# forestagostinelli/DeepCubeA

Measured on AMD Instinct MI355X. Metric: A* nodes expanded/sec on cube3, batch 20k, higher is better.
Workload: dtype u8 states / f64 cost keys / f32 heuristic

## Files before the change

deepcubea_amd/csrc/dca_engine.hip:

```cpp
#include <string.h>

#include <new>
#include <vector>

#include "dca_common.h"
#include "dca_tile.h"

namespace dca {

constexpr int NBIN = 4096;
constexpr int kBinsPerThread = NBIN / 1024;
constexpr int kLgNbin = 12;
constexpr int kSub = 2048;
constexpr int kScanBlocks = 256;
constexpr int kCollectBlocks = 512;
constexpr int kRankBlocks = 256;
constexpr uint32_t kTinyBin = 512;
constexpr int kSortCap = 8192;
constexpr int RT = 512;
constexpr int kRegEnt = 16;
constexpr uint32_t kLdsEnt = RT * kRegEnt;
constexpr int kStash = 2560;
constexpr int kSegs = NBIN + 1 + kSub;
constexpr uint32_t kGiantBin = 8192;
constexpr int kMaxLevels = 9;
constexpr unsigned long long kBarrierTimeout = 200000000ull;
constexpr unsigned long long kBarrierTimeoutFirst = 25000000ull;
constexpr uint32_t GBAR_BROKEN = 0x80000000u;
constexpr uint32_t NIL = 0xFFFFFFFFu;
constexpr uint32_t ID_MASK = 0x7FFFFFFFu, ID_SOLVED = 0x80000000u;
constexpr uint64_t EMPTY = ~0ull;
constexpr uint64_t DEAD = ~0ull;
constexpr uint32_t GINF = 0xFFFFFFFFu;
constexpr int kMaxMoves = 4096;

struct Slot {
    uint64_t entry;
    uint32_t g;
    uint32_t head;
};

struct alignas(128) Cnt {
    uint32_t v;
    uint32_t pad[31];
};
struct alignas(128) GRange {
    uint64_t kmin, kmax;
    uint32_t imin, imax;
    uint32_t pad[26];
};
struct alignas(128) Rng {
    uint64_t kmin, kmax;
    uint64_t pad[14];
};
struct IterState {
    uint32_t pool_n;
    uint32_t npop, m, base;
    uint32_t best_id;
    int32_t has_best;
    float best_cost;
};
struct Ctl {
    int32_t done, failed, stop_after, pad0;
    int64_t iters, gen, expanded;
    IterState S[2];
    uint32_t cur_f;
    uint32_t hbin;
    uint32_t front_above;
    uint32_t cur_b;
    uint64_t T;
    uint32_t refill, compact, r_bstar, spill_bin, r_move;
    uint64_t r_kmin;
    uint32_t r_shift;
    uint32_t want, bstar, shift, n_big, n_ord;
    uint32_t giant;
    uint32_t tseg;
    uint32_t pre_b, cn_star;
    uint64_t sel_kmin;
    uint32_t goal_id;
    uint32_t dbg_nord, dbg_maxbin, dbg_giant, dbg_giant_seen, dbg_maxsub;
    Cnt open_n[4];
    Cnt closed_n, back_dead, front_dead, ret_n, ticket_a;
    Cnt gbar;
    GRange grange;
    Rng rng[4];
    alignas(128) unsigned long long goal_best;
    alignas(128) uint32_t first_solved;
};

__device__ __forceinline__ uint64_t key_of_cost(double c) {
    uint64_t b = (uint64_t)__double_as_longlong(c);
    return (b & 0x8000000000000000ull) ? ~b : (b | 0x8000000000000000ull);
}
__device__ __forceinline__ double cost_of_key(uint64_t k) {
    uint64_t b = (k & 0x8000000000000000ull) ? (k & 0x7FFFFFFFFFFFFFFFull) : ~k;
    return __longlong_as_double((long long)b);
}
__device__ __forceinline__ uint32_t select_shift(uint64_t kmin, uint64_t kmax) {
    uint64_t range = kmax - kmin;
    int bits = range ? 64 - __clzll((long long)range) : 0;
    return bits > kLgNbin ? (uint32_t)(bits - kLgNbin) : 0u;
}
__device__ __forceinline__ uint32_t bin_of(uint64_t k, uint64_t kmin, uint32_t shift) {
    if (k <= kmin) return 0u;
    const uint64_t f = (k - kmin) >> shift;
    return f < (uint64_t)NBIN ? (uint32_t)f : (uint32_t)(NBIN - 1);
}
__device__ __forceinline__ bool pair_less(uint64_t ka, uint32_t ia, uint64_t kb, uint32_t ib) {
    return ka < kb || (ka == kb && (ia & ID_MASK) < (ib & ID_MASK));
}

enum {
    P_REFILL_HIST = 0, P_REFILL_SCAN, P_REFILL_MOVE, P_SEL_HIST, P_SEL_SCAN, P_SEL_COLLECT, P_RANK, P_EXPAND,
    P_PROBE,
    P_DECIDE, P_PACK, P_COMMIT, P_RANK_SMALL, P_RANK_BIG, P_RB_LOAD, P_RB_COUNT, P_RB_SCATTER, P_RB_ORDER, P_COUNT
};
constexpr int kProfSlots = 1024;
__device__ int g_back_squeeze_mark;
__device__ int g_first_barrier_gives_up;
__device__ __forceinline__ uint32_t rank_shares(uint32_t cn) {
    return cn <= (uint32_t)(512 * 16) ? (cn + 1023u) / 1024u : 1u;
}

#if defined(__HIP_DEVICE_COMPILE__)
#define DCA_GLOBAL __attribute__((address_space(1)))
#else
#define DCA_GLOBAL
#endif
template <class T>
using gp = T DCA_GLOBAL*;
template <class T>
using gr = T DCA_GLOBAL&;
typedef uint32_t __attribute__((aligned(1), may_alias)) unaligned_u32;
__device__ __forceinline__ uint32_t load_word(gp<const uint8_t> p) { return *(gp<const unaligned_u32>)p; }
template <class T, bool DEV>
struct EngPtr {
    typedef T* type;
};
template <class T>
struct EngPtr<T, true> {
    typedef gp<T> type;
};
template <class T>
__device__ __forceinline__ T* generic(gp<T> p) {
    return (T*)p;
}
using ::atomicAdd;
using ::atomicCAS;
using ::atomicExch;
using ::atomicMax;
using ::atomicMin;
template <class T, class V>
__device__ __forceinline__ T atomicAdd(gp<T> p, V v) {
    return ::atomicAdd(generic(p), (T)v);
}
template <class T, class V>
__device__ __forceinline__ T atomicMin(gp<T> p, V v) {
    return ::atomicMin(generic(p), (T)v);
}
template <class T, class V>
__device__ __forceinline__ T atomicMax(gp<T> p, V v) {
    return ::atomicMax(generic(p), (T)v);
}
template <class T, class V>
__device__ __forceinline__ T atomicExch(gp<T> p, V v) {
    return ::atomicExch(generic(p), (T)v);
}
template <class T, class U, class V>
__device__ __forceinline__ T atomicCAS(gp<T> p, U cmp, V v) {
    return ::atomicCAS(generic(p), (T)cmp, (T)v);
}

template <bool DEV>
struct EngT {
    template <class T>
// ... 677 lines not shown
    if (done) return;
    Stamp stamp(E, P_SEL_SCAN);
    uint32_t cb = cur0;
    uint64_t new_kmin = old_kmin;
    uint32_t new_shift = old_shift;
    if (rebased) {
        new_kmin = cur0 ? r1min : r0min;
        uint64_t kmax = cur0 ? r1max : r0max;
        if (T0 != ~0ull && T0 > kmax) kmax = T0;
        new_shift = kmax > new_kmin ? select_shift(new_kmin, kmax) : 0u;
        for (int o = 32; o > 0; o >>= 1) {
            const uint64_t a = __shfl_xor(mn, o), z = __shfl_xor(mx, o);
            mn = a < mn ? a : mn;
            mx = z > mx ? z : mx;
        }
        if ((t & 63) == 0) {
            s_red[0][t >> 6] = mn;
            s_red[1][t >> 6] = mx;
        }
        cb ^= 1;
    }
    if (t == 0) {
        s_maxbin = 0;
        s_giant = 0;
        s_nbig = 0;
        s_spill = NBIN;
        s_bstar = 0;
        s_hbin = NBIN;
    }
    scan_vals(hv, pre, wsum);
    const uint32_t n = rebased ? (cb ? on1 : on0) : (cb ? on1 : on0) - dead0 - above0;
    const uint32_t want = n < (uint32_t)E.B ? n : (uint32_t)E.B;
    const uint32_t hwant = (uint32_t)(kRefillPeriod + 2) * (uint32_t)E.B;
    for (int k = 0; k < kBinsPerThread; k++) {
        int bin = kBinsPerThread * t + k;
        if (pre[bin] < want && want <= pre[bin + 1]) s_bstar = (uint32_t)bin;
        if (rebased && n > E.f_max) {
            const uint32_t keepn = want + front_keep(E);
            if (pre[bin] < keepn && keepn <= pre[bin + 1]) s_spill = (uint32_t)bin;
        }
        if (rebased && pre[bin] < hwant && hwant <= pre[bin + 1]) s_hbin = (uint32_t)bin + 1u;
        E.pre[bin] = pre[bin];
        E.fill[bin] = 0;
    }
    for (int i = NBIN + t; i < kSegs; i += 1024) E.fill[i] = 0;
    if (t == 1023) E.pre[NBIN] = pre[NBIN];
    __syncthreads();
    const bool giant = E.coop && !coop_is_off(E) && want != 0 && pre[s_bstar + 1] - pre[s_bstar] > kGiantBin;
    if (giant)
        for (int i = t; i < kMaxLevels * kSub; i += 1024) E.subhist[i] = 0;
    for (int k = 0; k < kBinsPerThread; k++) {
        const uint32_t bin = kBinsPerThread * t + k;
        if (bin <= s_bstar && want != 0) {
            const uint32_t cn = pre[bin + 1] - pre[bin];
            if (cn > 256) atomicMax(&s_maxbin, cn);
            if (cn > (uint32_t)kSortCap) atomicAdd(&s_giant, 1u);
            if (cn > kTinyBin && !(giant && bin == s_bstar)) {
                uint32_t G = rank_shares(cn);
                G = G > 8u ? 8u : G;
                const uint32_t at = atomicAdd(&s_nbig, G);
                for (uint32_t g = 0; g < G; g++) E.big_list[at + g] = bin | (g << 16) | (G << 20);
            }
        }
    }
    __syncthreads();
    if (t == 0) {
        if (rebased) {
            uint64_t fmn = ~0ull, fmx = 0;
            for (int w = 0; w < 16; w++) {
                fmn = s_red[0][w] < fmn ? s_red[0][w] : fmn;
                fmx = s_red[1][w] > fmx ? s_red[1][w] : fmx;
            }
            c->cur_f = cb;
            c->rng[cb].kmin = fmn;
            c->rng[cb].kmax = fmx;
            c->hbin = s_hbin;
        }
        if (refill) {
            if (compact) {
                c->cur_b ^= 1;
                c->back_dead.v = 0;
                c->compact = 0;
            }
            c->refill = 0;
        }
        c->want = want;
        c->bstar = s_bstar;
        c->tseg = s_bstar;
        c->pre_b = pre[s_bstar];
        c->cn_star = pre[s_bstar + 1] - pre[s_bstar];
        c->giant = giant ? 1u : 0u;
        c->gbar.v = 0;
        c->grange.kmin = ~0ull;
        c->grange.kmax = 0;
        c->grange.imin = ~0u;
        c->grange.imax = 0;
        c->sel_kmin = new_kmin;
        c->shift = new_shift;
        uint32_t sp = s_spill;
        if (sp < NBIN - 1) {
            const uint64_t top = new_kmin + (((uint64_t)sp + 1) << new_shift) - 1;
            if (top >= new_kmin && top < T0) c->T = top;  else sp = NBIN;
        } else {
            sp = NBIN;
        }
        if (rebased) c->front_above = sp < NBIN ? pre[NBIN] - pre[sp + 1] : 0u;
        c->spill_bin = sp;
        s_sp = sp;
        c->goal_best = ~0ull;
        c->first_solved = NIL;
        if (want == 0) {
            c->failed = 1;
            c->done = 1;
        }
        c->n_big = s_nbig;
        c->n_ord = want ? pre[s_bstar + 1] : 0;
        c->ret_n.v = 0;
        c->dbg_maxsub = 0;
        c->front_dead.v = (rebased ? 0u : dead0) + want;
        c->dbg_nord = want ? pre[s_bstar + 1] : 0;
        c->dbg_maxbin = s_maxbin;
        c->dbg_giant = s_giant;
        c->dbg_giant_seen = giant_seen + s_giant;
    }
    __syncthreads();
    {
        const uint32_t bstar = s_bstar, sp = s_sp;
        for (int k = 0; k < kBinsPerThread; k++) {
            const uint32_t bin = kBinsPerThread * t + k;
            if (want == 0) break;
            if (bin < bstar || bin > sp)
                E.hist[bin] = 0;
            else if (bin == bstar)
                E.hist[bin] = pre[bin + 1] - want;
        }
    }
}

typedef unsigned __int128 u128;
__device__ __forceinline__ u128 comp_of(uint64_t key, uint32_t id) { return ((u128)key << 32) | (u128)(id & ID_MASK); }
__device__ __forceinline__ int clz128(u128 v) {
    uint64_t hi = (uint64_t)(v >> 64), lo = (uint64_t)v;
    return hi ? __clzll((long long)hi) : 64 + (lo ? __clzll((long long)lo) : 64);
}

constexpr int kStashG = 1536;
struct CollectLds {
    uint32_t pre[NBIN + 4];
    uint32_t lcnt[NBIN];
    union {
        struct {
            uint64_t st_key[kStash];
            uint32_t st_idx[kStash];
            uint16_t st_f[kStash];
            uint16_t nzf[kStash];
        } n;
        struct {
            uint32_t lcnt_ext[kSegs - NBIN + 3];
            uint32_t subpre[kSub + 4];
            uint64_t st_key[kStashG];
            uint32_t st_idx[kStashG];
            uint16_t st_f[kStashG];
            uint16_t nzf[kStashG];
        } g;
    } u;
    uint64_t red64[2][4];
    uint32_t red32[2][4];
    uint32_t wsum[4];
    uint32_t st_n, nz_n, ok, tsub, nb, bstar;
};
static_assert(sizeof(CollectLds) <= 80 * 1024, "two workgroups of k_sel_collect must fit one CU's LDS");
static_assert(offsetof(CollectLds, u) == offsetof(CollectLds, lcnt) + sizeof(uint32_t) * NBIN, "lcnt must run on into lcnt_ext");
static_assert(sizeof(uint64_t) * kStashG >= sizeof(uint32_t) * kSub, "sub-bin counters alias the giant stash");

struct SelParams {
    uint32_t b, n;
    uint64_t kmin;
    uint32_t shift;
    uint32_t want, bstar, pre_b, cn_star;
    bool giant;
};

enum { BAR_FAIL = 0, BAR_PASS = 1, BAR_BROKEN = 2 };
__device__ __forceinline__ int collect_grid_barrier(const Eng& E, gp<Ctl> c, CollectLds& L, uint32_t target, bool first) {
    asm volatile("s_waitcnt vmcnt(0)" ::: "memory");
    __syncthreads();
    if (threadIdx.x == 0) {
        __builtin_amdgcn_fence(__ATOMIC_RELEASE, "agent");
        asm volatile("s_waitcnt vmcnt(0)" ::: "memory");
        uint32_t v = __hip_atomic_fetch_add(&c->gbar.v, 1u, __ATOMIC_RELAXED, __HIP_MEMORY_SCOPE_AGENT) + 1u;
        int res = BAR_PASS;
        const unsigned long long t0 = wall_clock64();
        const unsigned long long limit = first ? (g_first_barrier_gives_up ? 0ull : kBarrierTimeoutFirst) : kBarrierTimeout;
        for (;;) {
            if (v & GBAR_BROKEN) {
                res = first ? BAR_BROKEN : BAR_FAIL;
                break;
            }
            if (v >= target) break;
            __builtin_amdgcn_s_sleep(4);
            if (__hip_atomic_load(&c->failed, __ATOMIC_RELAXED, __HIP_MEMORY_SCOPE_AGENT) != 0) {
                res = BAR_FAIL;
                break;
            }
            if (wall_clock64() - t0 > limit) {
                if (!first) {
                    res = BAR_FAIL;
                    break;
                }
                uint32_t expect = v;
                if (__hip_atomic_compare_exchange_strong(&c->gbar.v, &expect, v | GBAR_BROKEN, __ATOMIC_RELAXED, __ATOMIC_RELAXED,
                                                         __HIP_MEMORY_SCOPE_AGENT)) {
                    res = BAR_BROKEN;
                    break;
                }
                v = expect;
                continue;
            }
            v = __hip_atomic_load(&c->gbar.v, __ATOMIC_RELAXED, __HIP_MEMORY_SCOPE_AGENT);
        }
        __builtin_amdgcn_fence(__ATOMIC_ACQUIRE, "agent");
        if (res == BAR_FAIL) {
            __hip_atomic_store(&c->failed, 1, __ATOMIC_RELAXED, __HIP_MEMORY_SCOPE_AGENT);
            __hip_atomic_store(&c->done, 1, __ATOMIC_RELAXED, __HIP_MEMORY_SCOPE_AGENT);
        } else if (res == BAR_BROKEN) {
            __hip_atomic_store(E.coop_off, 1u, __ATOMIC_RELAXED, __HIP_MEMORY_SCOPE_AGENT);
        }
        L.ok = (uint32_t)res;
    }
    __syncthreads();
    return (int)L.ok;
}

__device__ __forceinline__ int collect_giant(const Eng& E, gp<Ctl> c, CollectLds& L, const SelParams P) {
    const uint32_t t = threadIdx.x, lane = t & 63, wv = t >> 6;
    const uint32_t n = P.n;
    const uint64_t bkmin = P.kmin;
    const uint32_t shift = P.shift, bstar = P.bstar, want = P.want;
    const uint32_t pre_b = P.pre_b;
    gp<uint64_t> __restrict__ keys = E.open_key[P.b];
    gp<const uint32_t> __restrict__ ids = E.open_id[P.b];
    constexpr uint32_t ITEMS = 8, TILE = 256 * ITEMS;
    const uint32_t ntiles = (n + TILE - 1) / TILE;
    uint32_t phase = 0;
    {
        uint64_t kmn = ~0ull, kmx = 0;
        uint32_t imn = ~0u, imx = 0;
        for (uint32_t tile = blockIdx.x; tile < ntiles; tile += gridDim.x) {
            uint64_t k[ITEMS];
            uint32_t id[ITEMS];
#pragma unroll
            for (uint32_t i = 0; i < ITEMS; i++) {
                const uint32_t idx = tile * TILE + i * 256 + t, ic = idx < n ? idx : n - 1;
                k[i] = keys[ic];
                id[i] = ids[ic] & ID_MASK;
                if (idx >= n) k[i] = DEAD;
            }
#pragma unroll
            for (uint32_t i = 0; i < ITEMS; i++) {
                const bool in = k[i] != DEAD && bin_of(k[i], bkmin, shift) == bstar;
                kmn = in && k[i] < kmn ? k[i] : kmn;
                kmx = in && k[i] > kmx ? k[i] : kmx;
                imn = in && id[i] < imn ? id[i] : imn;
                imx = in && id[i] > imx ? id[i] : imx;
            }
        }
        for (int o = 32; o > 0; o >>= 1) {
            const uint64_t a = __shfl_xor(kmn, o), z = __shfl_xor(kmx, o);
            const uint32_t x = __shfl_xor(imn, o), y = __shfl_xor(imx, o);
            kmn = a < kmn ? a : kmn;
            kmx = z > kmx ? z : kmx;
            imn = x < imn ? x : imn;
            imx = y > imx ? y : imx;
        }
        if (lane == 0) {
            L.red64[0][wv] = kmn;
            L.red64[1][wv] = kmx;
            L.red32[0][wv] = imn;
            L.red32[1][wv] = imx;
        }
        __syncthreads();
        if (t == 0) {
            for (int w = 1; w < 4; w++) {
                kmn = L.red64[0][w] < kmn ? L.red64[0][w] : kmn;
                kmx = L.red64[1][w] > kmx ? L.red64[1][w] : kmx;
                imn = L.red32[0][w] < imn ? L.red32[0][w] : imn;
                imx = L.red32[1][w] > imx ? L.red32[1][w] : imx;
            }
            if (kmn <= kmx) {
                atomicMin((unsigned long long*)&c->grange.kmin, (unsigned long long)kmn);
                atomicMax((unsigned long long*)&c->grange.kmax, (unsigned long long)kmx);
                atomicMin(&c->grange.imin, imn);
                atomicMax(&c->grange.imax, imx);
            }
        }
    }
    if (const int r = collect_grid_barrier(E, c, L, ++phase * gridDim.x, true); r != BAR_PASS) return r;
    const uint64_t gkmin = __hip_atomic_load(&c->grange.kmin, __ATOMIC_RELAXED, __HIP_MEMORY_SCOPE_AGENT);
    const uint64_t gkmax = __hip_atomic_load(&c->grange.kmax, __ATOMIC_RELAXED, __HIP_MEMORY_SCOPE_AGENT);
    const uint32_t gimin = __hip_atomic_load(&c->grange.imin, __ATOMIC_RELAXED, __HIP_MEMORY_SCOPE_AGENT);
    const uint32_t gimax = __hip_atomic_load(&c->grange.imax, __ATOMIC_RELAXED, __HIP_MEMORY_SCOPE_AGENT);
    u128 V0 = ((u128)gkmin << 32) + (u128)gimin;
    u128 span = ((u128)(gkmax - gkmin) << 32) + (u128)(gimax - gimin);
    uint32_t need = want - pre_b, below = 0, shc = 0, tsub = 0;
    uint32_t* lh = reinterpret_cast<uint32_t*>(L.u.g.st_key);
    uint32_t* subpre = L.u.g.subpre;
// ... 59 lines not shown
        if (cn <= kGiantBin || shc == 0 || lvl + 1 >= kMaxLevels) break;
        below += subpre[tsub];
        need -= subpre[tsub];
        V0 += (u128)tsub << shc;
        span = ((u128)1 << shc) - 1;
        __syncthreads();
    }
    const uint32_t seg0 = bstar + 1u;
    if (blockIdx.x == 0) {
        if (t == 0) {
            L.nb = c->n_big;
            E.pre[bstar + 1] = pre_b + below;
            c->tseg = seg0 + tsub;
            c->n_ord = pre_b + below + subpre[tsub + 1];
            c->dbg_nord = pre_b + below + subpre[tsub + 1];
        }
        __syncthreads();
        for (uint32_t sg = t; sg <= tsub + 1u; sg += 256) {
            const uint32_t cn = sg == 0 ? below : subpre[sg] - subpre[sg - 1];
            if (sg > 0) E.pre[seg0 + sg] = pre_b + below + subpre[sg];
            if (cn > kTinyBin) {
                uint32_t G = rank_shares(cn);
                G = G > 8u ? 8u : G;
                const uint32_t at = atomicAdd(&L.nb, G);
                for (uint32_t g = 0; g < G; g++) E.big_list[at + g] = (bstar + sg) | (g << 16) | (G << 20);
            }
        }
        __syncthreads();
        if (t == 0) c->n_big = L.nb;
    }
    uint32_t* lcnt = L.lcnt;
    for (uint32_t i = t; i < (uint32_t)(kSegs + 3); i += 256) lcnt[i] = 0;
    if (t == 0) {
        L.st_n = 0;
        L.nz_n = 0;
    }
    __syncthreads();
    uint64_t* st_key = L.u.g.st_key;
    uint32_t* st_idx = L.u.g.st_idx;
    uint16_t *st_f = L.u.g.st_f, *nzf = L.u.g.nzf;
    auto seg_base = [&](uint32_t f) -> uint32_t {
        return f < bstar ? L.pre[f] : f == bstar ? pre_b : pre_b + below + subpre[f - seg0];
    };
    auto seg_end = [&](uint32_t f) -> uint32_t {
        return f < bstar ? L.pre[f + 1] : f == bstar ? pre_b + below : pre_b + below + subpre[f - seg0 + 1];
    };
    auto flush = [&]() {
        const uint32_t ns = L.st_n < (uint32_t)kStashG ? L.st_n : (uint32_t)kStashG;
        const uint32_t nz = L.nz_n;
        for (uint32_t i = t; i < nz; i += 256) {
            const uint32_t f = nzf[i];
            lcnt[f] = atomicAdd(&E.fill[f], lcnt[f]);
        }
        __syncthreads();
        for (uint32_t p = t; p < ns; p += 256) {
            const uint32_t f = st_f[p];
            const uint32_t id = ids[st_idx[p]];
            const uint32_t pos = seg_base(f) + atomicAdd(&lcnt[f], 1u);
            if (pos < seg_end(f)) {
                E.tmp_key[pos] = st_key[p];
                E.tmp_id[pos] = id;
                E.tmp_f[pos] = (uint16_t)f;
                E.tmp_idx[pos] = st_idx[p];
            } else {
                c->failed = 1;
            }
        }
        __syncthreads();
        for (uint32_t i = t; i < nz; i += 256) lcnt[nzf[i]] = 0;
        __syncthreads();
        if (t == 0) {
            L.st_n = 0;
            L.nz_n = 0;
        }
        __syncthreads();
    };
    constexpr uint32_t ITEMS_D = 4, TILE_D = 256 * ITEMS_D;
    const uint32_t ntiles_d = (n + TILE_D - 1) / TILE_D;
    for (uint32_t tile2 = blockIdx.x; tile2 < ntiles; tile2 += gridDim.x) {
        for (uint32_t half = 0; half < 2; half++) {
            const uint32_t tile = tile2 * 2 + half;
            if (tile < ntiles_d) {
                uint64_t k[ITEMS_D];
                uint32_t id[ITEMS_D];
#pragma unroll
                for (uint32_t i = 0; i < ITEMS_D; i++) {
                    const uint32_t idx = tile * TILE_D + i * 256 + t, ic = idx < n ? idx : n - 1;
                    k[i] = keys[ic];
                    id[i] = ids[ic];
                    if (idx >= n) k[i] = DEAD;
                }
#pragma unroll
                for (uint32_t i = 0; i < ITEMS_D; i++) {
                    if (k[i] == DEAD) continue;
                    uint32_t f = bin_of(k[i], bkmin, shift);
                    if (f > bstar) continue;
                    if (f == bstar) {
                        const u128 v = comp_of(k[i], id[i]);
                        if (v >= V0) {
                            if (v - V0 > span) continue;
                            const uint32_t sub = (uint32_t)((v - V0) >> shc);
                            if (sub > tsub) continue;
                            f = seg0 + sub;
                        }
                    }
                    const uint32_t idx = tile * TILE_D + i * 256 + t;
                    const uint32_t p = atomicAdd(&L.st_n, 1u);
                    keys[idx] = DEAD;
                    if (p < (uint32_t)kStashG) {
                        st_key[p] = k[i];
                        st_idx[p] = idx;
                        st_f[p] = (uint16_t)f;
                        if (atomicAdd(&lcnt[f], 1u) == 0u) nzf[atomicAdd(&L.nz_n, 1u)] = (uint16_t)f;
                    } else {
                        const uint32_t pos = seg_base(f) + atomicAdd(&E.fill[f], 1u);
                        if (pos < seg_end(f)) {
                            E.tmp_key[pos] = k[i];
                            E.tmp_id[pos] = id[i];
                            E.tmp_f[pos] = (uint16_t)f;
                            E.tmp_idx[pos] = idx;
                        } else {
                            c->failed = 1;
                        }
                    }
                }
            }
            __syncthreads();
            if (L.st_n + TILE_D > (uint32_t)kStashG) flush();
        }
    }
    __syncthreads();
    flush();
    return BAR_PASS;
}

template <bool FUSED>
__global__ __launch_bounds__(256) void k_sel_collect(const Eng* __restrict__ engs) {
    const Eng& E = engs[blockIdx.y];
    gp<Ctl> c = E.ctl;
    if (c->done) return;
    Stamp stamp(E, P_SEL_COLLECT);
    extern __shared__ __attribute__((aligned(16))) uint8_t collect_lds[];
    CollectLds& L = *reinterpret_cast<CollectLds*>(collect_lds);
    const uint32_t t = threadIdx.x;
    SelParams P;
    {
        const uint32_t b = c->cur_f, on0 = c->open_n[0].v, on1 = c->open_n[1].v;
        P.b = b;
        P.n = b ? on1 : on0;
        P.kmin = c->sel_kmin;
        P.shift = c->shift;
        P.want = c->want;
    }
    if constexpr (FUSED) {
        constexpr int PER = NBIN / 256;
        const uint32_t lane = t & 63, wv = t >> 6;
        uint32_t v[PER], sum = 0;
        {
            const uint4* h4 = reinterpret_cast<const uint4*>(E.hist + PER * t);
#pragma unroll
            for (int q = 0; q < PER / 4; q++) {
                const uint4 x = h4[q];
                v[4 * q] = x.x;
                v[4 * q + 1] = x.y;
                v[4 * q + 2] = x.z;
                v[4 * q + 3] = x.w;
            }
#pragma unroll
            for (int k = 0; k < PER; k++) sum += v[k];
        }
        uint32_t incl = sum;
        for (int o = 1; o < 64; o <<= 1) {
            const uint32_t u = __shfl_up(incl, o);
            if (lane >= (uint32_t)o) incl += u;
        }
        if (lane == 63) L.wsum[wv] = incl;
        if (t == 0) L.bstar = 0;
        __syncthreads();
        uint32_t run = incl - sum;
        for (uint32_t w = 0; w < wv; w++) run += L.wsum[w];
        const uint32_t want = P.want;
#pragma unroll
        for (int k = 0; k < PER; k++) {
            L.pre[PER * t + k] = run;
            if (run < want && want <= run + v[k]) L.bstar = PER * t + k;
            run += v[k];
        }
        if (t == 255) L.pre[NBIN] = run;
        __syncthreads();
        if (want == 0) {
            if (blockIdx.x == 0 && t == 0) {
                c->failed = 1;
                c->done = 1;
            }
            return;
        }
        P.bstar = L.bstar;
        P.pre_b = L.pre[P.bstar];
        P.cn_star = L.pre[P.bstar + 1] - P.pre_b;
        P.giant = E.coop && !coop_is_off(E) && P.cn_star > kGiantBin;
        if (blockIdx.x == 0) {
            for (uint32_t i = t; i <= (uint32_t)NBIN; i += 256) E.pre[i] = L.pre[i];
            if (t == 0) {
                L.nb = 0;
                L.st_n = 0;
                L.nz_n = 0;
            }
            __syncthreads();
            for (uint32_t bin = t; bin <= P.bstar; bin += 256) {
                const uint32_t cn = L.pre[bin + 1] - L.pre[bin];
                if (cn > 256) atomicMax(&L.st_n, cn);
                if (cn > (uint32_t)kSortCap) atomicAdd(&L.nz_n, 1u);
                if (cn > kTinyBin && !(P.giant && bin == P.bstar)) {
                    uint32_t G = rank_shares(cn);
                    G = G > 8u ? 8u : G;
                    const uint32_t at = atomicAdd(&L.nb, G);
                    for (uint32_t g = 0; g < G; g++) E.big_list[at + g] = bin | (g << 16) | (G << 20);
                }
            }
            __syncthreads();
            if (t == 0) {
                c->bstar = P.bstar;
                c->tseg = P.bstar;
                c->giant = P.giant ? 1u : 0u;
                c->pre_b = P.pre_b;
                c->cn_star = P.cn_star;
                c->spill_bin = NBIN;
                c->n_big = L.nb;
                c->n_ord = L.pre[P.bstar + 1];
                c->front_dead.v += want;
                c->dbg_nord = L.pre[P.bstar + 1];
                c->dbg_maxbin = L.st_n;
                c->dbg_giant = L.nz_n;
                c->dbg_giant_seen += L.nz_n;
                c->dbg_maxsub = 0;
            }
            __syncthreads();
        }
    } else {
        P.bstar = c->bstar;
        P.giant = c->giant != 0;
        P.pre_b = c->pre_b;
        P.cn_star = c->cn_star;
        if (P.want == 0) return;
        for (uint32_t i = t; i <= P.bstar + 1u; i += 256) L.pre[i] = E.pre[i];
        __syncthreads();
    }
    if (P.giant) {
        if (collect_giant(E, c, L, P) != BAR_BROKEN) return;
        if (blockIdx.x == 0 && t == 0) {
            const uint32_t cn = P.cn_star;
            uint32_t G = rank_shares(cn);
            G = G > 8u ? 8u : G;
            const uint32_t at = c->n_big;
            if (cn > kTinyBin) {
                for (uint32_t g = 0; g < G; g++) E.big_list[at + g] = P.bstar | (g << 16) | (G << 20);
                c->n_big = at + G;
            }
            c->giant = 0;
        }
        P.giant = false;
        __syncthreads();
    }
    const uint32_t n = P.n;
    const uint64_t kmin = P.kmin;
    const uint32_t shift = P.shift, bstar = P.bstar;
    gp<uint64_t> __restrict__ keys = E.open_key[P.b];
    gp<const uint32_t> __restrict__ ids = E.open_id[P.b];
    constexpr uint32_t ITEMS = 8, TILE = 256 * ITEMS;
    const uint32_t ntiles = (n + TILE - 1) / TILE;
    uint64_t* st_key = L.u.n.st_key;
    uint32_t* st_idx = L.u.n.st_idx;
    uint16_t *st_f = L.u.n.st_f, *nzf = L.u.n.nzf;
    for (int i = t; i < NBIN; i += 256) L.lcnt[i] = 0;
    if (t == 0) {
        L.st_n = 0;
        L.nz_n = 0;
    }
    __syncthreads();
    auto flush = [&]() {
        const uint32_t ns = L.st_n < (uint32_t)kStash ? L.st_n : (uint32_t)kStash;
        const uint32_t nz = L.nz_n;
        for (uint32_t i = t; i < nz; i += 256) {
            const uint32_t f = nzf[i];
            L.lcnt[f] = atomicAdd(&E.fill[f], L.lcnt[f]);
        }
        __syncthreads();
        for (uint32_t p = t; p < ns; p += 256) {
            const uint32_t f = st_f[p];
            const uint32_t id = ids[st_idx[p]];
            const uint32_t pos = L.pre[f] + atomicAdd(&L.lcnt[f], 1u);
            if (pos < L.pre[f + 1]) {
                E.tmp_key[pos] = st_key[p];
                E.tmp_id[pos] = id;
                E.tmp_f[pos] = (uint16_t)f;
                E.tmp_idx[pos] = st_idx[p];
            } else {
                c->failed = 1;
            }
        }
        __syncthreads();
        for (uint32_t i = t; i < nz; i += 256) L.lcnt[nzf[i]] = 0;
        __syncthreads();
        if (t == 0) {
            L.st_n = 0;
            L.nz_n = 0;
        }
        __syncthreads();
    };
    for (uint32_t tile = blockIdx.x; tile < ntiles; tile += gridDim.x) {
        uint64_t k[ITEMS];
        uint32_t dest = 0;
#pragma unroll
        for (uint32_t i = 0; i < ITEMS; i++) {
            const uint32_t idx = tile * TILE + i * 256 + t, ic = idx < n ? idx : n - 1;
            k[i] = keys[ic];
            if (idx >= n) k[i] = DEAD;
        }
#pragma unroll
        for (uint32_t i = 0; i < ITEMS; i++) {
            const uint32_t f = bin_of(k[i], kmin, shift);
            const uint32_t d = (k[i] != DEAD && f <= bstar) ? 1u : 0u;
            dest |= d << (2 * i);
        }
        if (dest & 0x5555u & ~(dest >> 1)) {
#pragma unroll
            for (uint32_t i = 0; i < ITEMS; i++) {
                if (((dest >> (2 * i)) & 3u) != 1u) continue;
                const uint32_t idx = tile * TILE + i * 256 + t;
                const uint32_t f = bin_of(k[i], kmin, shift);
                const uint32_t p = atomicAdd(&L.st_n, 1u);
                keys[idx] = DEAD;
                if (p < kStash) {
                    st_key[p] = k[i];
                    st_idx[p] = idx;
                    st_f[p] = (uint16_t)f;
                    if (atomicAdd(&L.lcnt[f], 1u) == 0u) nzf[atomicAdd(&L.nz_n, 1u)] = (uint16_t)f;
                } else {
                    const uint32_t pos = L.pre[f] + atomicAdd(&E.fill[f], 1u);
                    if (pos < L.pre[f + 1]) {
                        E.tmp_key[pos] = k[i];
                        E.tmp_id[pos] = ids[idx];
                        E.tmp_f[pos] = (uint16_t)f;
                        E.tmp_idx[pos] = idx;
                    } else {
                        c->failed = 1;
                    }
                }
            }
        }
        __syncthreads();
        if (L.st_n + TILE > (uint32_t)kStash) flush();
    }
    __syncthreads();
    flush();
}


constexpr int kRankStack = 512;
constexpr uint32_t kDirectMax = 512;
constexpr uint32_t kSubMax = 512;

struct RankItem {
    uint32_t off, n, need, src;
    uint32_t g, G;
    uint32_t nopush;
};
struct RankShared {
    uint32_t cnt[kSub + 64];
    uint32_t off[kSub + 1];
    uint32_t wsum[16];
    uint64_t red_lo[32], red_hi[32];
    uint64_t vmin_hi, vmin_lo;
    uint64_t kmin, kspan;
    uint32_t imin, ispan;
    uint32_t bits, tsub, sp, fail;
    uint32_t ret_base, ret_cnt;
    RankItem stack[kRankStack];
};

__device__ __forceinline__ void emit_pop(const Eng& E, gp<Ctl> c, uint32_t rank, uint64_t key, uint32_t id) {
    E.pop_key[rank] = key;
    E.pop_id[rank] = id;
    if (id & ID_SOLVED) {
        if (E.sem == DCA_SEM_PY)
            atomicMin(&c->goal_best, ((unsigned long long)(uint32_t)E.g[id & ID_MASK] << 32) | rank);
        else
            atomicMin(&c->first_solved, rank);
    }
}
__device__ __forceinline__ void emit_ranked(const Eng& E, gp<Ctl> c, uint32_t nf, bool live, uint32_t rank, uint32_t want,
                                            uint64_t key, uint32_t id) {
    if (live && rank < want) emit_pop(E, c, rank, key, id);
    const bool back = live && rank >= want;
    const unsigned long long mask = __ballot(back);
    if (mask == 0) return;
    const int lane = threadIdx.x & 63;
    const int leader = __ffsll((long long)mask) - 1;
    uint32_t basep = 0;
    if (lane == leader) basep = atomicAdd(&c->ret_n.v, (uint32_t)__popcll(mask));
    basep = __shfl(basep, leader);
    if (back) {
        const uint32_t slot = E.tmp_idx[basep + (uint32_t)__popcll(mask & ((1ull << lane) - 1ull))];
        E.open_key[nf][slot] = key;
        E.open_id[nf][slot] = id;
    }
}
__device__ __forceinline__ void ret_begin(gp<Ctl> c, RankShared& S, uint32_t nf, uint32_t count) {
    __syncthreads();
    if (threadIdx.x == 0) {
        S.ret_base = count ? atomicAdd(&c->ret_n.v, count) : 0u;
        S.ret_cnt = 0;
    }
    __syncthreads();
}
struct RetAcc {};
__device__ __forceinline__ void ret_put(const Eng& E, gp<Ctl> c, RankShared& S, uint32_t nf, bool pred, uint64_t key,
                                        uint32_t id, RetAcc& acc) {
    const unsigned long long mask = __ballot(pred);
    if (mask == 0) return;
    const int lane = threadIdx.x & 63;
    const int leader = __ffsll((long long)mask) - 1;
    uint32_t basep = 0;
    if (lane == leader) basep = atomicAdd(&S.ret_cnt, (uint32_t)__popcll(mask));
    basep = __shfl(basep, leader);
    if (pred) {
        const uint32_t slot = E.tmp_idx[S.ret_base + basep + (uint32_t)__popcll(mask & ((1ull << lane) - 1ull))];
        E.open_key[nf][slot] = key;
        E.open_id[nf][slot] = id;
    }
}
__device__ __forceinline__ void ret_end(gp<Ctl> c, uint32_t nf, RetAcc acc) {}
template <int NJ>
__device__ __forceinline__ void ret_put_many(const Eng& E, RankShared& S, uint32_t nf, uint32_t n_ord, uint32_t preds,
                                             const uint64_t* key, const uint32_t* id) {
    const uint32_t cnt = (uint32_t)__popc(preds);
    const int lane = threadIdx.x & 63;
    uint32_t incl = cnt;
    for (int o = 1; o < 64; o <<= 1) {
        const uint32_t u = __shfl_up(incl, o);
        if (lane >= o) incl += u;
    }
    const uint32_t total = __shfl(incl, 63);
    if (total == 0) return;
    uint32_t basep = 0;
    if (lane == 63) basep = atomicAdd(&S.ret_cnt, total);
    basep = __shfl(basep, 63);
    uint32_t r = S.ret_base + basep + incl - cnt;
    uint32_t slot[NJ];
#pragma unroll
    for (int j = 0; j < NJ; j++) {
        slot[j] = E.tmp_idx[r < n_ord ? r : n_ord - 1];
        r += (preds >> j) & 1u;
    }
#pragma unroll
    for (int j = 0; j < NJ; j++)
        if ((preds >> j) & 1u) {
            E.open_key[nf][slot[j]] = key[j];
            E.open_id[nf][slot[j]] = id[j];
        }
}

__device__ __forceinline__ void rank_small_entries(const Eng& E, gp<Ctl> c, RankShared& S, uint64_t* LK, uint32_t* LI,
                                                   uint32_t nf, uint32_t p0, uint32_t n_ord, uint32_t want) {
    const uint32_t t = threadIdx.x;
    const uint32_t plast = (p0 + RT - 1 < n_ord ? p0 + RT - 1 : n_ord - 1);
    const uint32_t f_lo = E.tmp_f[p0], f_hi = E.tmp_f[plast];
    const uint32_t lo = E.pre[f_lo], hi = E.pre[f_hi + 1];
    const bool staged = hi - lo <= kLdsEnt && f_hi - f_lo + 2 <= (uint32_t)kSub;
    if (staged) {
        for (uint32_t i = t; i < hi - lo; i += RT) {
            LK[i] = E.tmp_key[lo + i];
            LI[i] = E.tmp_id[lo + i];
        }
        for (uint32_t i = t; i < f_hi - f_lo + 2; i += RT) S.off[i] = E.pre[f_lo + i];
    }
    __syncthreads();
    const uint32_t p = p0 + t;
    bool live = p < n_ord;
    uint64_t k = 0;
    uint32_t id = 0, rank = 0;
    if (live) {
        const uint32_t f = E.tmp_f[p];
        const uint32_t o = staged ? S.off[f - f_lo] : E.pre[f], e = staged ? S.off[f - f_lo + 1] : E.pre[f + 1];
        if (e - o > kTinyBin) {
            live = false;
        } else if (staged) {
            k = LK[p - lo];
            id = LI[p - lo];
            rank = o;
            for (uint32_t j = o - lo; j < e - lo; j++) rank += pair_less(LK[j], LI[j], k, id) ? 1u : 0u;
        } else {
            k = E.tmp_key[p];
            id = E.tmp_id[p];
            rank = o;
            for (uint32_t j = o; j < e; j++) rank += pair_less(E.tmp_key[j], E.tmp_id[j], k, id) ? 1u : 0u;
        }
    }
    emit_ranked(E, c, nf, live, rank, want, k, id);
    __syncthreads();
}

__device__ __forceinline__ uint32_t sub_of(uint64_t k, uint32_t id, u128 vmin, uint32_t shc, uint32_t nsub) {
    const u128 q = (comp_of(k, id) - vmin) >> shc;
    return q < (u128)nsub ? (uint32_t)q : nsub - 1u;
}


// ... 2191 lines not shown
```

Before: 102.7 million.

## Double-buffer key/id prefetch in selection collect and stash ids in LDS

Restructures the k_sel_collect tile loop into two register buffers of keys and ids. The first two sets are fetched before the histogram scan and later sets are prefetched while the current one is processed, so global load latency overlaps the scan and the binning work. Open-list ids are now loaded alongside keys and stored in a new LDS stash array, which removes the dependent gather in flush. To fit LDS the stash shrinks, and the tile-to-block mapping becomes interleaved, which adds register pressure and may cause more frequent flushes.

```diff
diff --git a/deepcubea_amd/csrc/dca_engine.hip b/deepcubea_amd/csrc/dca_engine.hip
--- a/deepcubea_amd/csrc/dca_engine.hip
+++ b/deepcubea_amd/csrc/dca_engine.hip
@@ -20,7 +20,7 @@
 constexpr int RT = 512;
 constexpr int kRegEnt = 16;
 constexpr uint32_t kLdsEnt = RT * kRegEnt;
-constexpr int kStash = 2560;
+constexpr int kStash = 2432;
 constexpr int kSegs = NBIN + 1 + kSub;
 constexpr uint32_t kGiantBin = 8192;
 constexpr int kMaxLevels = 9;
@@ -1004,6 +1004,7 @@
         struct {
             uint64_t st_key[kStash];
             uint32_t st_idx[kStash];
+            uint32_t st_id[kStash];
             uint16_t st_f[kStash];
             uint16_t nzf[kStash];
         } n;
@@ -1369,19 +1370,39 @@
         P.shift = c->shift;
         P.want = c->want;
     }
+    constexpr uint32_t ITEMS = 8, TILE = 256 * ITEMS;
+    const uint32_t G = gridDim.x;
+    const uint32_t n = P.n, nsets = (n + TILE * G - 1) / (TILE * G), i_last = n ? n - 1 : 0;
+    gp<uint64_t> __restrict__ keys = E.open_key[P.b];
+    gp<const uint32_t> __restrict__ ids = E.open_id[P.b];
+    uint64_t ka[ITEMS], kb[ITEMS];
+    uint32_t ia[ITEMS], ib[ITEMS];
+    auto at = [&](uint32_t set, uint32_t i) { return ((set * ITEMS + i) * G + blockIdx.x) * 256 + t; };
+    auto fetch = [&](uint64_t(&k)[ITEMS], uint32_t(&id)[ITEMS], uint32_t set) {
+#pragma unroll
+        for (uint32_t i = 0; i < ITEMS; i++) {
+            const uint32_t idx = at(set, i), ic = idx < n ? idx : i_last;
+            k[i] = keys[ic];
+            id[i] = ids[ic];
+        }
+    };
     if constexpr (FUSED) {
         constexpr int PER = NBIN / 256;
         const uint32_t lane = t & 63, wv = t >> 6;
         uint32_t v[PER], sum = 0;
         {
             const uint4* h4 = reinterpret_cast<const uint4*>(E.hist + PER * t);
+            uint4 x[PER / 4];
+#pragma unroll
+            for (int q = 0; q < PER / 4; q++) x[q] = h4[q];
+            fetch(ka, ia, 0);
+            fetch(kb, ib, 1);
 #pragma unroll
             for (int q = 0; q < PER / 4; q++) {
-                const uint4 x = h4[q];
-                v[4 * q] = x.x;
-                v[4 * q + 1] = x.y;
-                v[4 * q + 2] = x.z;
-                v[4 * q + 3] = x.w;
+                v[4 * q] = x[q].x;
+                v[4 * q + 1] = x[q].y;
+                v[4 * q + 2] = x[q].z;
+                v[4 * q + 3] = x[q].w;
             }
 #pragma unroll
             for (int k = 0; k < PER; k++) sum += v[k];
@@ -1415,7 +1436,7 @@
         P.bstar = L.bstar;
         P.pre_b = L.pre[P.bstar];
         P.cn_star = L.pre[P.bstar + 1] - P.pre_b;
-        P.giant = E.coop && !coop_is_off(E) && P.cn_star > kGiantBin;
+        P.giant = P.cn_star > kGiantBin && E.coop && !coop_is_off(E);
         if (blockIdx.x == 0) {
             for (uint32_t i = t; i <= (uint32_t)NBIN; i += 256) E.pre[i] = L.pre[i];
             if (t == 0) {
@@ -1460,6 +1481,8 @@
         P.pre_b = c->pre_b;
         P.cn_star = c->cn_star;
         if (P.want == 0) return;
+        fetch(ka, ia, 0);
+        fetch(kb, ib, 1);
         for (uint32_t i = t; i <= P.bstar + 1u; i += 256) L.pre[i] = E.pre[i];
         __syncthreads();
     }
@@ -1478,16 +1501,13 @@
         }
         P.giant = false;
         __syncthreads();
-    }
-    const uint32_t n = P.n;
+        fetch(ka, ia, 0);
+        fetch(kb, ib, 1);
+    }
     const uint64_t kmin = P.kmin;
     const uint32_t shift = P.shift, bstar = P.bstar;
-    gp<uint64_t> __restrict__ keys = E.open_key[P.b];
-    gp<const uint32_t> __restrict__ ids = E.open_id[P.b];
-    constexpr uint32_t ITEMS = 8, TILE = 256 * ITEMS;
-    const uint32_t ntiles = (n + TILE - 1) / TILE;
     uint64_t* st_key = L.u.n.st_key;
-    uint32_t* st_idx = L.u.n.st_idx;
+    uint32_t *st_idx = L.u.n.st_idx, *st_id = L.u.n.st_id;
     uint16_t *st_f = L.u.n.st_f, *nzf = L.u.n.nzf;
     for (int i = t; i < NBIN; i += 256) L.lcnt[i] = 0;
     if (t == 0) {
@@ -1495,7 +1515,7 @@
         L.nz_n = 0;
     }
     __syncthreads();
-    auto flush = [&]() {
+    auto flush = [&](bool last) {
         const uint32_t ns = L.st_n < (uint32_t)kStash ? L.st_n : (uint32_t)kStash;
         const uint32_t nz = L.nz_n;
         for (uint32_t i = t; i < nz; i += 256) {
@@ -1505,17 +1525,17 @@
         __syncthreads();
         for (uint32_t p = t; p < ns; p += 256) {
             const uint32_t f = st_f[p];
-            const uint32_t id = ids[st_idx[p]];
             const uint32_t pos = L.pre[f] + atomicAdd(&L.lcnt[f], 1u);
             if (pos < L.pre[f + 1]) {
                 E.tmp_key[pos] = st_key[p];
-                E.tmp_id[pos] = id;
+                E.tmp_id[pos] = st_id[p];
                 E.tmp_f[pos] = (uint16_t)f;
                 E.tmp_idx[pos] = st_idx[p];
             } else {
                 c->failed = 1;
             }
         }
+        if (last) return;
         __syncthreads();
         for (uint32_t i = t; i < nz; i += 256) L.lcnt[nzf[i]] = 0;
         __syncthreads();
@@ -1525,32 +1545,27 @@
         }
         __syncthreads();
     };
-    for (uint32_t tile = blockIdx.x; tile < ntiles; tile += gridDim.x) {
-        uint64_t k[ITEMS];
+    auto pass = [&](const uint64_t(&k)[ITEMS], const uint32_t(&id)[ITEMS], uint32_t set) {
         uint32_t dest = 0;
 #pragma unroll
         for (uint32_t i = 0; i < ITEMS; i++) {
-            const uint32_t idx = tile * TILE + i * 256 + t, ic = idx < n ? idx : n - 1;
-            k[i] = keys[ic];
-            if (idx >= n) k[i] = DEAD;
-        }
-#pragma unroll
-        for (uint32_t i = 0; i < ITEMS; i++) {
+            const uint32_t idx = at(set, i);
             const uint32_t f = bin_of(k[i], kmin, shift);
-            const uint32_t d = (k[i] != DEAD && f <= bstar) ? 1u : 0u;
+            const uint32_t d = (idx < n && k[i] != DEAD && f <= bstar) ? 1u : 0u;
             dest |= d << (2 * i);
         }
         if (dest & 0x5555u & ~(dest >> 1)) {
 #pragma unroll
             for (uint32_t i = 0; i < ITEMS; i++) {
                 if (((dest >> (2 * i)) & 3u) != 1u) continue;
-                const uint32_t idx = tile * TILE + i * 256 + t;
+                const uint32_t idx = at(set, i);
                 const uint32_t f = bin_of(k[i], kmin, shift);
                 const uint32_t p = atomicAdd(&L.st_n, 1u);
                 keys[idx] = DEAD;
                 if (p < kStash) {
                     st_key[p] = k[i];
                     st_idx[p] = idx;
+                    st_id[p] = id[i];
                     st_f[p] = (uint16_t)f;
                     if (atomicAdd(&L.lcnt[f], 1u) == 0u) nzf[atomicAdd(&L.nz_n, 1u)] = (uint16_t)f;
                 } else {
@@ -1566,11 +1581,24 @@
                 }
             }
         }
+    };
+    auto make_room = [&]() {
+        const uint32_t have = L.st_n;
         __syncthreads();
-        if (L.st_n + TILE > (uint32_t)kStash) flush();
-    }
-    __syncthreads();
-    flush();
+        if (have + TILE > (uint32_t)kStash) flush(false);
+    };
+    for (uint32_t set = 0; set < nsets; set += 2) {
+        pass(ka, ia, set);
+        fetch(ka, ia, set + 2);
+        __syncthreads();
+        if (set + 1 >= nsets) break;
+        make_room();
+        pass(kb, ib, set + 1);
+        fetch(kb, ib, set + 3);
+        __syncthreads();
+        if (set + 2 < nsets) make_room();
+    }
+    flush(true);
 }
 
 
```

Measured after the change: 102.7 million. No clear change (-0.0%).
